# NeptuneHub/AudioMuse-AI

Hardware: AMD Instinct MI355X
Metric: clap_clips_per_sec (higher is better)
Workload: dtype bf16; 1 GPU; model=htsat_clap_student_49M, global_batch=256, seq_len=480000, parallelism=dp1

## Files before the change

audiomuse_amd/config.py:

```python

from __future__ import annotations

import os
from typing import Callable, Dict, Optional

_DB_OVERRIDE_PROVIDER: Optional[Callable[[], Dict[str, str]]] = None


def _env(name: str, default: str) -> str:
    return os.environ.get(name, default)


def _env_int(name: str, default: int) -> int:
    try:
        return int(os.environ.get(name, default))
    except (TypeError, ValueError):
        return default


def _env_float(name: str, default: float) -> float:
    try:
        return float(os.environ.get(name, default))
    except (TypeError, ValueError):
        return default
# ... 253 lines not shown
    "CLUSTERING_STALL_TIMEOUT_MINUTES", 30.0)
TOP_N_ELITES = _env_int("TOP_N_ELITES", 5)
EXPLOITATION_START_FRACTION = _env_float("EXPLOITATION_START_FRACTION", 0.2)
EXPLOITATION_PROBABILITY_CONFIG = _env_float(
    "EXPLOITATION_PROBABILITY_CONFIG", 0.6)
MUTATION_INT_ABS_DELTA = _env_int("MUTATION_INT_ABS_DELTA", 3)
MUTATION_FLOAT_ABS_DELTA = _env_float("MUTATION_FLOAT_ABS_DELTA", 0.25)
MUTATION_KMEANS_COORD_FRACTION = _env_float(
    "MUTATION_KMEANS_COORD_FRACTION", 0.05)
SAMPLING_PERCENTAGE_CHANGE_PER_RUN = _env_float(
    "SAMPLING_PERCENTAGE_CHANGE_PER_RUN", 0.2)
MIN_SONGS_PER_GENRE_FOR_STRATIFICATION = _env_int(
    "MIN_SONGS_PER_GENRE_FOR_STRATIFICATION", 100)
STRATIFIED_SAMPLING_TARGET_PERCENTILE = _env_float(
    "STRATIFIED_SAMPLING_TARGET_PERCENTILE", 50.0)
TOP_K_MOODS_FOR_PURITY_CALCULATION = _env_int(
    "TOP_K_MOODS_FOR_PURITY_CALCULATION", 3)
CLUSTER_NAMING_AI_HISTORY = _env_bool("CLUSTER_NAMING_AI_HISTORY", True)
PLAYLIST_NAME_HISTORY_ROUNDS = _env_int("PLAYLIST_NAME_HISTORY_ROUNDS", 3)

NUM_CLUSTERS_MIN = _env_int("NUM_CLUSTERS_MIN", 2)
NUM_CLUSTERS_MAX = _env_int("NUM_CLUSTERS_MAX", 40)
DBSCAN_EPS_MIN = _env_float("DBSCAN_EPS_MIN", 0.2)
DBSCAN_EPS_MAX = _env_float("DBSCAN_EPS_MAX", 2.5)
DBSCAN_MIN_SAMPLES_MIN = _env_int("DBSCAN_MIN_SAMPLES_MIN", 3)
DBSCAN_MIN_SAMPLES_MAX = _env_int("DBSCAN_MIN_SAMPLES_MAX", 15)
GMM_N_COMPONENTS_MIN = _env_int("GMM_N_COMPONENTS_MIN", 2)
GMM_N_COMPONENTS_MAX = _env_int("GMM_N_COMPONENTS_MAX", 30)
GMM_COVARIANCE_TYPE = _env("GMM_COVARIANCE_TYPE", "diag")
SPECTRAL_N_CLUSTERS_MIN = _env_int("SPECTRAL_N_CLUSTERS_MIN", 2)
SPECTRAL_N_CLUSTERS_MAX = _env_int("SPECTRAL_N_CLUSTERS_MAX", 30)
SPECTRAL_N_NEIGHBORS = _env_int("SPECTRAL_N_NEIGHBORS", 10)
PCA_COMPONENTS_MIN = _env_int("PCA_COMPONENTS_MIN", 0)
PCA_COMPONENTS_MAX = _env_int("PCA_COMPONENTS_MAX", 32)

SCORE_WEIGHT_DIVERSITY = _env_float("SCORE_WEIGHT_DIVERSITY", 2.0)
SCORE_WEIGHT_PURITY = _env_float("SCORE_WEIGHT_PURITY", 1.0)
SCORE_WEIGHT_OTHER_FEATURE_DIVERSITY = _env_float(
    "SCORE_WEIGHT_OTHER_FEATURE_DIVERSITY", 0.0)
SCORE_WEIGHT_OTHER_FEATURE_PURITY = _env_float(
    "SCORE_WEIGHT_OTHER_FEATURE_PURITY", 0.0)
SCORE_WEIGHT_SILHOUETTE = _env_float("SCORE_WEIGHT_SILHOUETTE", 0.0)
SCORE_WEIGHT_DAVIES_BOULDIN = _env_float("SCORE_WEIGHT_DAVIES_BOULDIN", 0.0)
SCORE_WEIGHT_CALINSKI_HARABASZ = _env_float(
    "SCORE_WEIGHT_CALINSKI_HARABASZ", 0.0)

SEM_GROVE_LYRICS_WEIGHT = _env_float("SEM_GROVE_LYRICS_WEIGHT", 0.75)
SEM_GROVE_AUDIO_WEIGHT = _env_float("SEM_GROVE_AUDIO_WEIGHT", 0.25)

ARTIST_GMM_MIN_COMPONENTS = 2
ARTIST_GMM_MAX_COMPONENTS = 10
INDEX_BUILD_WORKERS = _env_int("INDEX_BUILD_WORKERS", 4)

SONIC_FINGERPRINT_HALF_LIFE_DAYS = _env_float("SONIC_FINGERPRINT_HALF_LIFE_DAYS", 30.0)
SONIC_FINGERPRINT_TOP_PLAYED = _env_int("SONIC_FINGERPRINT_TOP_PLAYED", 100)
SONIC_FINGERPRINT_TOP_N_SONGS = _env_int("SONIC_FINGERPRINT_TOP_N_SONGS", 50)
SONIC_FINGERPRINT_NEIGHBORS = _env_int("SONIC_FINGERPRINT_NEIGHBORS", 3)
SONIC_FINGERPRINT_MAX_SONGS_PER_ALBUM = _env_int(
    "SONIC_FINGERPRINT_MAX_SONGS_PER_ALBUM", 0)
SONIC_FINGERPRINT_CRON_PLAYLIST_NAME = _env(
    "SONIC_FINGERPRINT_CRON_PLAYLIST_NAME", "Sonic Fingerprint_automatic")

HYPERBOLIC_SCALE_PERCENTILE = _env_float("HYPERBOLIC_SCALE_PERCENTILE", 95.0)
HYPERBOLIC_DEFAULT_LIMIT = _env_int("HYPERBOLIC_DEFAULT_LIMIT", 50)
HYPERBOLIC_MAX_LIMIT = _env_int("HYPERBOLIC_MAX_LIMIT", 500)
HYPERBOLIC_RADIAL_SPREAD = _env_float("HYPERBOLIC_RADIAL_SPREAD", 0.8)
HYPERBOLIC_CANDIDATE_OVERFETCH = _env_int("HYPERBOLIC_CANDIDATE_OVERFETCH", 4)
HYPERBOLIC_RADIUS_SCALE = _env_float("HYPERBOLIC_RADIUS_SCALE", 1.0)
HYPERBOLIC_RADIUS_PERCENTILE = _env_float("HYPERBOLIC_RADIUS_PERCENTILE", 95.0)
HYPERBOLIC_TARGET_LEAF_SIZE = _env_int("HYPERBOLIC_TARGET_LEAF_SIZE", 200)
HYPERBOLIC_MIN_CLUSTER_SIZE = _env_int("HYPERBOLIC_MIN_CLUSTER_SIZE", 10)
HYPERBOLIC_TREE_WARMUP_DURATION = _env_float(
    "HYPERBOLIC_TREE_WARMUP_DURATION", 300.0)

RADIUS_WALK_BUCKETS = _env_int("RADIUS_WALK_BUCKETS", 10)
RADIUS_INSTRUMENTATION = _env_bool("RADIUS_INSTRUMENTATION", False)

GPU_DTYPE = _env("GPU_DTYPE", "bf16")
CLAP_GPU_BATCH = _env_int("CLAP_GPU_BATCH", 256)
CLAP_FP8_SERVING = _env_bool("AUDIOMUSE_FP8_SERVING", False)
FP8_HIDDEN_ENABLE = _env_bool("AUDIOMUSE_FP8_HIDDEN", False)
FP8_ATTN_ENABLE = _env_bool("AUDIOMUSE_FP8_ATTN", False)
MLP_FUSED_ENABLE = _env_bool("AUDIOMUSE_MLP_FUSED", True)
MERGE_LN_GATHER = _env_bool("AUDIOMUSE_MERGE_LN_GATHER", True)
HIP_REQUIRE_NATIVE = _env_bool("HIP_REQUIRE_NATIVE", True)
RCCL_BUCKET_CAP_MB = _env_int("RCCL_BUCKET_CAP_MB", 64)

AI_PROVIDER = _env("AI_MODEL_PROVIDER", _env("AI_PROVIDER", "none"))
AI_MODEL_NAME = _env("AI_MODEL_NAME", "")
AI_BASE_URL = _env("AI_BASE_URL", "")
AI_API_KEY = _env("AI_API_KEY", "")
AI_MAX_TOOL_CALLS = _env_int("AI_MAX_TOOL_CALLS", 4)
AI_REQUEST_TIMEOUT_SECONDS = _env_float("AI_REQUEST_TIMEOUT_SECONDS", 60.0)
MAX_SONGS_IN_AI_PROMPT = _env_int("MAX_SONGS_IN_AI_PROMPT", 100)
AI_TOOLCALL_TEMPERATURE = _env_float("AI_TOOLCALL_TEMPERATURE", 0.2)
AI_TOOLCALL_TOP_P = _env_float("AI_TOOLCALL_TOP_P", 0.9)
AI_TOOLCALL_TOP_K = _env_int("AI_TOOLCALL_TOP_K", 40)
AI_TOOLCALL_MIN_P = _env_float("AI_TOOLCALL_MIN_P", 0.0)
AI_TOOLCALL_NUM_PREDICT = _env_int("AI_TOOLCALL_NUM_PREDICT", 1024)
OPENAI_API_KEY = _env("OPENAI_API_KEY", "no-key-needed")
OPENAI_MODEL_NAME = _env("OPENAI_MODEL_NAME", "gpt-4o-mini")
OPENAI_SERVER_URL = _env("OPENAI_SERVER_URL", "https://api.openai.com/v1")
OLLAMA_SERVER_URL = _env("OLLAMA_SERVER_URL", "http://127.0.0.1:11434/v1")
OLLAMA_MODEL_NAME = _env("OLLAMA_MODEL_NAME", "llama3.1")
GEMINI_API_KEY = _env("GEMINI_API_KEY", "")
GEMINI_MODEL_NAME = _env("GEMINI_MODEL_NAME", "gemini-2.0-flash")
MISTRAL_API_KEY = _env("MISTRAL_API_KEY", "")
MISTRAL_MODEL_NAME = _env("MISTRAL_MODEL_NAME", "mistral-small-latest")

PLUGINS_ENABLED = _env_bool("PLUGINS_ENABLED", True)
PLUGIN_MAX_DOWNLOAD_MB = _env_int("PLUGIN_MAX_DOWNLOAD_MB", 50)
PLUGIN_ALLOW_PIP = _env_bool("PLUGIN_ALLOW_PIP", False)

JWT_SECRET = _env("AUDIOMUSE_JWT_SECRET", _env("JWT_SECRET", ""))
API_TOKEN = _env("AUDIOMUSE_API_TOKEN", _env("API_TOKEN", ""))
AUTH_ENABLED = _env_bool("AUTH_ENABLED", True)
AUDIOMUSE_USER = _env("AUDIOMUSE_USER", "")
AUDIOMUSE_PASSWORD = _env("AUDIOMUSE_PASSWORD", "")
BEHIND_PROXY = _env_bool("ENABLE_PROXY_FIX",
                         _env_bool("AUDIOMUSE_BEHIND_PROXY", False))
DASHBOARD_BROWSE_PAGE_SIZE = _env_int("DASHBOARD_BROWSE_PAGE_SIZE", 100)
DASHBOARD_BROWSE_MAX_OFFSET = _env_int("DASHBOARD_BROWSE_MAX_OFFSET", 10000)
DASHBOARD_REFRESH_SECONDS = _env_float("DASHBOARD_REFRESH_SECONDS", 60.0)


def set_db_override_provider(provider: Optional[Callable[[], Dict[str, str]]]) -> None:
    global _DB_OVERRIDE_PROVIDER
    _DB_OVERRIDE_PROVIDER = provider


def apply_db_overrides(overrides: Dict[str, str]) -> int:
    import sys

    module = sys.modules[__name__]
    applied = 0
    for key, raw in (overrides or {}).items():
        if not key.isupper() or not hasattr(module, key):
            continue
        current = getattr(module, key)
        try:
            if isinstance(current, bool):
                value = str(raw).strip().lower() in ("1", "true", "yes", "on")
            elif isinstance(current, int):
                value = int(raw)
            elif isinstance(current, float):
                value = float(raw)
            elif isinstance(current, str):
                value = str(raw)
            else:
                continue
        except (TypeError, ValueError):
            continue
        setattr(module, key, value)
        applied += 1
    return applied


def refresh_config() -> None:
    if _DB_OVERRIDE_PROVIDER is not None:
        apply_db_overrides(_DB_OVERRIDE_PROVIDER() or {})


_DEFAULTS_SNAPSHOT: Dict[str, object] = {
    _k: _v for _k, _v in list(globals().items())
    if _k.isupper() and isinstance(_v, (bool, int, float, str))
}
# ... 5 lines not shown
```

audiomuse_amd/models/htsat.py:

```python

from __future__ import annotations

from dataclasses import dataclass
from typing import List, Tuple

import torch
import torch.nn as nn
import torch.nn.functional as F

from audiomuse_amd.ops.attention import window_attention
from audiomuse_amd.ops.norms import FusedLayerNorm


@dataclass
class HTSATConfig:
    n_mels: int = 128
    n_frames: int = 1024
    patch_size: int = 4
    embed_dim: int = 128
    depths: Tuple[int, ...] = (2, 2, 6, 2)
    num_heads: Tuple[int, ...] = (4, 8, 16, 32)
    window: int = 8
    mlp_ratio: float = 4.0
    out_dim: int = 512
# ... 5 lines not shown
    x = x.view(B, H // w, w, W // w, w, C)
    return x.permute(0, 1, 3, 2, 4, 5).reshape(-1, w * w, C)


def window_reverse(win: torch.Tensor, w: int, H: int, W: int) -> torch.Tensor:
    B = win.shape[0] // (H // w * W // w)
    x = win.view(B, H // w, W // w, w, w, -1)
    return x.permute(0, 1, 3, 2, 4, 5).reshape(B, H, W, -1)


class WindowAttention(nn.Module):

    def __init__(self, dim: int, heads: int, window: int):
        super().__init__()
        self.dim = dim
        self.heads = heads
        self.window = window
        self.scale = (dim // heads) ** -0.5
        self.qkv = nn.Linear(dim, dim * 3, bias=True)
        self.proj = nn.Linear(dim, dim)

        n = (2 * window - 1) ** 2
        self.rel_bias = nn.Parameter(torch.zeros(n, heads))
        coords = torch.stack(torch.meshgrid(
            torch.arange(window), torch.arange(window), indexing="ij"))
        flat = coords.flatten(1)
        rel = flat[:, :, None] - flat[:, None, :]
        rel = rel.permute(1, 2, 0) + (window - 1)
        idx = rel[..., 0] * (2 * window - 1) + rel[..., 1]
        self.register_buffer("rel_index", idx, persistent=False)
        nn.init.trunc_normal_(self.rel_bias, std=0.02)

    def full_bias(self) -> torch.Tensor:
        T = self.window * self.window
        bias = self.rel_bias[self.rel_index.view(-1)].view(T, T, self.heads)
        return bias.permute(2, 0, 1).float().contiguous()

    def full_bias_bf16(self) -> torch.Tensor:
        ver = self.rel_bias._version
        cached = getattr(self, "_bias_cache", None)
        if cached is not None and cached[0] == ver \
                and cached[1].device == self.rel_bias.device:
            return cached[1]
        table = self.full_bias().to(torch.bfloat16).contiguous()
        self._bias_cache = (ver, table)
        return table

    def forward(self, x: torch.Tensor, mask: torch.Tensor | None) -> torch.Tensor:
        nW, T, C = x.shape
        qkv = self.qkv(x).reshape(nW, T, 3, self.heads, C // self.heads)
        q, k, v = qkv.permute(2, 0, 3, 1, 4).unbind(0)
        bias = self.full_bias().to(x.dtype)
        out = window_attention(q, k, v, bias, mask, self.scale)
        out = out.transpose(1, 2).reshape(nW, T, C)
        return self.proj(out)


class SwinBlock(nn.Module):
    def __init__(self, dim: int, heads: int, window: int, shift: int, mlp_ratio: float):
        super().__init__()
        self.window = window
        self.shift = shift
        self.norm1 = FusedLayerNorm(dim)
        self.attn = WindowAttention(dim, heads, window)
        self.norm2 = FusedLayerNorm(dim)
        hidden = int(dim * mlp_ratio)
        self.mlp = nn.Sequential(nn.Linear(dim, hidden),
                                 nn.GELU(approximate="tanh"),
                                 nn.Linear(hidden, dim))

    def _fused_available(self, x: torch.Tensor) -> bool:
        if not (x.is_cuda and x.dtype == torch.bfloat16
                and self.mlp[0].weight.dtype == torch.bfloat16
                and not torch.is_grad_enabled()):
            return False
        from audiomuse_amd.ops import _ext
        ext = _ext.native_or_none()
        return ext is not None and hasattr(ext, "window_attn_fwd")

    def _fused_attn_available(self, x: torch.Tensor) -> bool:
        return (self._fused_available(x) and self.window in (4, 8)
                and self.attn.heads % 2 == 0
                and self.attn.dim // self.attn.heads == 32)

    _MLP_FUSED_DIMS = (128,)
    _MLP_FUSED_BM = 128

    def _mlp_half(self, ext, x: torch.Tensor,
                  attn_out: torch.Tensor) -> torch.Tensor:
        from audiomuse_amd import config
        C = x.shape[-1]
        ln_w = self.norm2.weight.to(torch.bfloat16).contiguous()
        ln_b = self.norm2.bias.to(torch.bfloat16).contiguous()
        if (config.MLP_FUSED_ENABLE and C in self._MLP_FUSED_DIMS
                and self.mlp[0].out_features == 4 * C
                and (x.numel() // C) % self._MLP_FUSED_BM == 0):
            return ext.mlp_fused(
                x.contiguous(), attn_out.contiguous(), ln_w, ln_b,
                self.norm2.eps,
                self.mlp[0].weight.contiguous(), self.mlp[0].bias.contiguous(),
                self.mlp[2].weight.contiguous(), self.mlp[2].bias.contiguous())
        x2, xn2 = ext.add_layernorm_bf16(
            x.contiguous(), attn_out.contiguous(), ln_w, ln_b, self.norm2.eps)
        hidden = ext.linear_gelu(xn2, self.mlp[0].weight.contiguous(),
                                 self.mlp[0].bias.contiguous())
        return ext.linear_bias_add(hidden,
                                   self.mlp[2].weight.contiguous(),
                                   self.mlp[2].bias.contiguous(), x2)

    def _eager_attn(self, x: torch.Tensor, H: int, W: int,
                    mask: torch.Tensor | None) -> torch.Tensor:
        B, L, C = x.shape
        x = self.norm1(x).view(B, H, W, C)
        if self.shift:
            x = torch.roll(x, shifts=(-self.shift, -self.shift), dims=(1, 2))
        win = window_partition(x, self.window)
        win = self.attn(win, mask if self.shift else None)
        x = window_reverse(win, self.window, H, W)
        if self.shift:
            x = torch.roll(x, shifts=(self.shift, self.shift), dims=(1, 2))
        return x.view(B, L, C)

    def forward(self, x: torch.Tensor, H: int, W: int,
                mask: torch.Tensor | None) -> torch.Tensor:
        B, L, C = x.shape
        if self._fused_attn_available(x):
            from audiomuse_amd.ops import _ext, fp8
            ext = _ext.require()
            use_fp8 = fp8.serving_enabled() and fp8.available(x.device)
            out = None
            if use_fp8:
                xq, xs = fp8.ln_fp8(self.norm1, x)
                wq, ws = fp8.quantize_weight(self.attn.qkv.weight)
                qkv_bias = self.attn.qkv.bias.to(torch.bfloat16).contiguous()
                if self.window == 8 and fp8.FP8_ATTN[0]:
                    try:
                        qsc, qinv, qamax = fp8.hidden_state(self.attn.qkv,
                                                            x.device)
                        qkv8 = ext.linear_fp8(xq, wq, xs, ws, qkv_bias,
                                              d_inv_scale=qinv)
                        samp = qkv8.reshape(-1)[: 1 << 22]
                        qamax.copy_(samp.float().abs().amax() * qsc)
                        out = ext.window_attn_fp8_fwd(
                            qkv8.view(B, H, W, 3 * C),
                            self.attn.full_bias_bf16(), qsc,
                            self.attn.heads, self.shift, self.attn.scale)
                    except RuntimeError as exc:
                        fp8.FP8_ATTN[0] = False
                        fp8.FP8_ATTN_ERR = str(exc)
                if out is None:
                    qkv = ext.linear_fp8(xq, wq, xs, ws, qkv_bias)
            else:
                xn = self.norm1(x)
                qkv = ext.linear_bias(xn.contiguous(),
                                      self.attn.qkv.weight.contiguous(),
                                      self.attn.qkv.bias.contiguous())
            if out is None:
                attn_fwd = (ext.window_attn_fwd if self.window == 8
                            else ext.window_attn4_fwd)
                out = attn_fwd(
                    qkv.view(B, H, W, 3 * C), self.attn.full_bias_bf16(),
                    self.attn.heads, self.shift, self.attn.scale)
            out = out.view(B, L, C)
            proj = ext.linear_bias(out.contiguous(),
                                   self.attn.proj.weight.contiguous(),
                                   self.attn.proj.bias.contiguous())
            if use_fp8:
                x2, xn2q, xs2 = fp8.add_ln_fp8(self.norm2, x, proj)
                w0q, w0s = fp8.quantize_weight(self.mlp[0].weight)
                b0 = self.mlp[0].bias.to(torch.bfloat16).contiguous()
                if fp8.FP8_HIDDEN[0]:
                    try:
                        hs, hinv, hamax = fp8.hidden_state(self.mlp[0],
                                                           x.device)
                        hidden8 = ext.linear_fp8(xn2q, w0q, xs2, w0s, b0,
                                                 gelu=True,
                                                 d_inv_scale=hinv)
                        samp = hidden8.reshape(-1)[: 1 << 22]
                        hamax.copy_(samp.float().abs().amax() * hs)
                        w2q, w2s = fp8.quantize_weight(self.mlp[2].weight)
                        return ext.linear_fp8(
                            hidden8, w2q, hs, w2s,
                            self.mlp[2].bias.to(torch.bfloat16).contiguous(),
                            resid=x2)
                    except RuntimeError as exc:
                        fp8.FP8_HIDDEN[0] = False
                        fp8.FP8_HIDDEN_ERR = str(exc)
                hidden = ext.linear_fp8(xn2q, w0q, xs2, w0s, b0, gelu=True)
                return ext.linear_bias_add(hidden,
                                           self.mlp[2].weight.contiguous(),
                                           self.mlp[2].bias.contiguous(), x2)
            return self._mlp_half(ext, x, proj)
        if self._fused_available(x):
            from audiomuse_amd.ops import _ext
            ext = _ext.require()
            attn_out = self._eager_attn(x, H, W, mask)
            return self._mlp_half(ext, x, attn_out)
        x = x + self._eager_attn(x, H, W, mask)
        return x + self.mlp(self.norm2(x))


class PatchMerging(nn.Module):

    def __init__(self, dim: int):
        super().__init__()
        self.norm = FusedLayerNorm(4 * dim)
        self.reduction = nn.Linear(4 * dim, 2 * dim, bias=False)

    def _gather_available(self, x: torch.Tensor) -> bool:
        from audiomuse_amd import config
        if not (config.MERGE_LN_GATHER and x.is_cuda
                and x.dtype == torch.bfloat16
                and not torch.is_grad_enabled()
                and 128 < self.norm.normalized_shape[0] <= 4096):
            return False
        from audiomuse_amd.ops import _ext
        ext = _ext.native_or_none()
        return ext is not None and hasattr(ext, "merge_layernorm_bf16")

    def forward(self, x: torch.Tensor, H: int, W: int) -> torch.Tensor:
        B, L, C = x.shape
        if self._gather_available(x):
            from audiomuse_amd.ops import _ext
            y = _ext.require().merge_layernorm_bf16(
                x.contiguous().view(B, H, W, C),
                self.norm.weight.to(torch.bfloat16).contiguous(),
                self.norm.bias.to(torch.bfloat16).contiguous(),
                self.norm.eps)
            return self.reduction(y)
        x = x.view(B, H // 2, 2, W // 2, 2, C)
        x = x.permute(0, 1, 3, 4, 2, 5).reshape(B, (H // 2) * (W // 2),
                                                4 * C)
        return self.reduction(self.norm(x))

# ... 82 lines not shown
```

audiomuse_amd/ops/csrc/bindings.cpp:

```cpp
#include <hip/hip_runtime.h>
#include <torch/extension.h>

#include <algorithm>
#include <vector>

#include <c10/hip/HIPStream.h>

namespace audiomuse {
void launch_mel_fwd(const float* audio, float* out, const float* window,
                    const float2* twiddle, const int* mel_rowptr,
                    const int* mel_bin, const float* mel_w, int B, int T,
                    int n_frames, int hop, int n_mels, int n_fft, int center,
                    int log_mode, int quant16, hipStream_t stream);
void launch_ivf_scan(int dtype_code, int metric, const void* query,
                     const float* qnorm, const void* data,
                     const float* row_norm, const int* probe,
                     const int* cell_off, const long long* cand_off,
                     float* out_dist, int* out_row, int Q, int d, int nprobe,
                     long long cap, hipStream_t stream);
void launch_ivf_scan_sel(int dtype_code, int metric, const void* query,
                         const float* qnorm, const void* data,
                         const float* row_norm, const int* probe,
                         const int* sel_rows, const int* sel_off,
                         const long long* cand_off, float* out_dist,
                         int* out_row, int Q, int d, int nprobe, long long cap,
                         hipStream_t stream);
void launch_ivf_scan_topk(int dtype_code, int metric, const void* query,
                          const float* qnorm, const void* data,
                          const float* row_norm, const int* probe,
                          const int* off, const int* sel_rows,
                          const int* skip_row, float* out_dist, int* out_row,
                          int Q, int S, int K, int d, int nprobe,
                          hipStream_t stream);
void launch_umap_epoch(const float* E, float* out, const int* idx,
                       const int* thr, const int* in_off, const int* in_edge,
                       const int* in_thr, int n, int k, int n_in, int neg,
                       float alpha, float a, float b, unsigned int seed,
                       unsigned int epoch, hipStream_t stream);
void launch_path_relax(const float* dist_in, const int* pred_in,
                       float* dist_out, int* pred_out, const int* idx,
                       const float* w, const int* in_off, const int* in_edge,
                       const unsigned char* allowed, int* changed, int B,
                       int n, int k, int n_in, int legs_inner,
                       hipStream_t stream);
void launch_path_walk(const float* dist, const int* pred, const int* src,
                      const int* dst, int* out, int* count, int B, int n,
                      int T1, int legs_inner, hipStream_t stream);
void launch_layernorm_bf16(const void* x, void* y, const void* w,
                           const void* b, long long n_rows, int dim, float eps,
                           hipStream_t stream);
void launch_add_layernorm_bf16(const void* x, const void* in2, void* sum_out,
                               void* y, const void* w, const void* b,
                               long long n_rows, int dim, float eps,
                               hipStream_t stream);
void launch_layernorm_bf16_fp8_impl(const void* x, void* y8, const void* w,
                                    const void* b, const void* in2,
                                    void* sum_out, const float* q_scale,
                                    float* q_amax, long long n_rows, int dim,
                                    float eps, hipStream_t stream);
void launch_mfma_probe(const void* A, const void* B, float* D,
                       hipStream_t stream);
void launch_window_attn4(const void* qkv, void* out, const void* bias,
                         int Bn, int H, int W, int C, int heads, int shift,
                         float scale, hipStream_t stream);
void launch_window_attn(const void* qkv, void* out, const void* bias, int Bn,
                        int H, int W, int C, int heads, int shift, float scale,
                        hipStream_t stream);
void launch_merge_layernorm_bf16(const void* x, void* y, const void* w,
                                 const void* b, int Bn, int H, int W, int C,
                                 float eps, hipStream_t stream);
void launch_mlp_fused_c128(const void* x, const void* proj, const void* ln_w,
                           const void* ln_b, const void* W1, const void* b1,
                           const void* W2, const void* b2, void* out,
                           long long M, float eps, hipStream_t stream);
void launch_window_attn_fp8(const void* qkv, void* out, const void* bias,
                            const void* qs_ptr, int Bn, int H, int W, int C,
                            int heads, int shift, float sm_scale,
                            hipStream_t stream);
void launch_fp_align(const int* words, const long long* off, const int* pairs,
                     int* out, long long W, int F, long long P, int max_offset,
                     int min_words, int lds_words, hipStream_t stream);
}

#define AM_CHECK(x, msg) TORCH_CHECK(x, msg)
#define AM_CHECK_GPU_F32_CONTIG(t)                                   \
  TORCH_CHECK(t.is_cuda() && t.scalar_type() == at::kFloat &&        \
                  t.is_contiguous(),                                 \
              #t " must be a contiguous float32 GPU tensor")

static torch::Tensor mel_fwd(torch::Tensor audio, torch::Tensor window,
                             torch::Tensor twiddle, torch::Tensor mel_rowptr,
                             torch::Tensor mel_bin, torch::Tensor mel_w,
                             int64_t hop, int64_t n_fft, bool center,
                             int64_t log_mode, bool quant16) {
  AM_CHECK_GPU_F32_CONTIG(audio);
  AM_CHECK_GPU_F32_CONTIG(window);
  AM_CHECK_GPU_F32_CONTIG(mel_w);
  AM_CHECK(audio.dim() == 2, "audio must be (B, T)");
  AM_CHECK(twiddle.is_cuda() && twiddle.is_contiguous() &&
               twiddle.scalar_type() == at::kFloat &&
               twiddle.numel() == n_fft,
           "twiddle must be (n_fft/2, 2) float32 on GPU");
  AM_CHECK(mel_rowptr.is_cuda() && mel_rowptr.scalar_type() == at::kInt &&
               mel_bin.scalar_type() == at::kInt,
           "CSR index tensors must be int32 on GPU");
  AM_CHECK(n_fft == 256 || n_fft == 512 || n_fft == 1024 || n_fft == 2048 ||
               n_fft == 4096,
           "n_fft must be a power of two in [256, 4096]");

  const int64_t B = audio.size(0);
  const int64_t T = audio.size(1);
  const int64_t n_mels = mel_rowptr.numel() - 1;
  const int64_t n_frames =
      center ? (1 + T / hop) : (1 + (T - n_fft) / hop);
  AM_CHECK(n_frames >= 1, "audio too short for one frame");

  auto out = torch::empty({B, n_mels, n_frames}, audio.options());
  auto stream = c10::hip::getCurrentHIPStream();
  audiomuse::launch_mel_fwd(
      audio.data_ptr<float>(), out.data_ptr<float>(), window.data_ptr<float>(),
      reinterpret_cast<const float2*>(twiddle.data_ptr<float>()),
      mel_rowptr.data_ptr<int>(), mel_bin.data_ptr<int>(),
      mel_w.data_ptr<float>(), (int)B, (int)T, (int)n_frames, (int)hop,
      (int)n_mels, (int)n_fft, center ? 1 : 0, (int)log_mode, quant16 ? 1 : 0,
      stream.stream());
  C10_HIP_CHECK(hipGetLastError());
  return out;
}

static void ivf_scan(int64_t dtype_code, int64_t metric, torch::Tensor query,
                     torch::Tensor qnorm, torch::Tensor data,
                     torch::Tensor row_norm, torch::Tensor probe,
                     torch::Tensor cell_off, torch::Tensor cand_off,
                     torch::Tensor out_dist, torch::Tensor out_row,
                     int64_t dim_pad) {
  AM_CHECK(query.is_cuda() && data.is_cuda(), "ivf_scan needs GPU tensors");
  AM_CHECK(probe.scalar_type() == at::kInt && cell_off.scalar_type() == at::kInt,
           "probe/cell_off must be int32");
  AM_CHECK(cand_off.scalar_type() == at::kLong, "cand_off must be int64");
  AM_CHECK(out_dist.is_contiguous() && out_row.is_contiguous(),
           "outputs must be contiguous");
  const int Q = probe.size(0);
  const int nprobe = probe.size(1);
  const long long cap = out_dist.size(1);
  auto stream = c10::hip::getCurrentHIPStream();
  audiomuse::launch_ivf_scan(
      (int)dtype_code, (int)metric, query.data_ptr(), qnorm.data_ptr<float>(),
      data.data_ptr(), row_norm.data_ptr<float>(), probe.data_ptr<int>(),
      cell_off.data_ptr<int>(),
      reinterpret_cast<const long long*>(cand_off.data_ptr<int64_t>()),
      out_dist.data_ptr<float>(), out_row.data_ptr<int>(), Q, (int)dim_pad,
      nprobe, cap, stream.stream());
  C10_HIP_CHECK(hipGetLastError());
}

static void ivf_scan_sel(int64_t dtype_code, int64_t metric,
                         torch::Tensor query, torch::Tensor qnorm,
// ... 441 lines not shown
  return y8;
}

static std::vector<torch::Tensor> add_layernorm_bf16_fp8(
    torch::Tensor x, torch::Tensor other, torch::Tensor w, torch::Tensor b,
    double eps, torch::Tensor scale, torch::Tensor amax) {
  AM_CHECK(x.is_cuda() && x.scalar_type() == at::kBFloat16 && x.is_contiguous(),
           "x must be contiguous bf16 on GPU");
  AM_CHECK(other.is_contiguous() && other.sizes() == x.sizes() &&
               other.scalar_type() == at::kBFloat16,
           "other must match x");
  const int dim = x.size(-1);
  AM_CHECK(dim % 4 == 0 && dim <= 4096, "dim must be /4 and <= 4096");
  auto sum = torch::empty_like(x);
  auto y8 = torch::empty(x.sizes(), x.options().dtype(at::kFloat8_e4m3fn));
  const long long n_rows = x.numel() / dim;
  auto stream = c10::hip::getCurrentHIPStream();
  audiomuse::launch_layernorm_bf16_fp8_impl(
      x.data_ptr(), y8.data_ptr(), w.data_ptr(), b.data_ptr(),
      other.data_ptr(), sum.data_ptr(), scale.data_ptr<float>(),
      amax.data_ptr<float>(), n_rows, dim, (float)eps, stream.stream());
  C10_HIP_CHECK(hipGetLastError());
  return {sum, y8};
}

static torch::Tensor merge_layernorm_bf16(torch::Tensor x, torch::Tensor w,
                                          torch::Tensor b, double eps) {
  AM_CHECK(x.is_cuda() && x.scalar_type() == at::kBFloat16 &&
               x.is_contiguous() && x.dim() == 4,
           "x must be (B, H, W, C) bf16 contiguous GPU");
  const int64_t Bn = x.size(0), H = x.size(1), W = x.size(2), C = x.size(3);
  AM_CHECK(H % 2 == 0 && W % 2 == 0, "H, W must be even");
  AM_CHECK(C % 4 == 0 && 4 * C > 128 && 4 * C <= 4096,
           "C must be a multiple of 4 with 128 < 4C <= 4096");
  AM_CHECK(w.is_cuda() && b.is_cuda() && w.is_contiguous() &&
               b.is_contiguous() && w.scalar_type() == at::kBFloat16 &&
               b.scalar_type() == at::kBFloat16 && w.numel() == 4 * C &&
               b.numel() == 4 * C,
           "w/b must be contiguous bf16 of size 4C");
  auto y = torch::empty({Bn, (H / 2) * (W / 2), 4 * C}, x.options());
  auto stream = c10::hip::getCurrentHIPStream();
  audiomuse::launch_merge_layernorm_bf16(x.data_ptr(), y.data_ptr(),
                                         w.data_ptr(), b.data_ptr(), (int)Bn,
                                         (int)H, (int)W, (int)C, (float)eps,
                                         stream.stream());
  C10_HIP_CHECK(hipGetLastError());
  return y;
}

static torch::Tensor mlp_fused(torch::Tensor x, torch::Tensor proj,
                               torch::Tensor ln_w, torch::Tensor ln_b,
                               double eps, torch::Tensor w1, torch::Tensor b1,
                               torch::Tensor w2, torch::Tensor b2) {
  auto ok = [](const torch::Tensor& t) {
    return t.is_cuda() && t.scalar_type() == at::kBFloat16 &&
           t.is_contiguous();
  };
  AM_CHECK(ok(x) && ok(proj) && ok(ln_w) && ok(ln_b) && ok(w1) && ok(b1) &&
               ok(w2) && ok(b2),
           "all inputs must be contiguous bf16 GPU tensors");
  const int64_t C = x.size(-1);
  AM_CHECK(C == 128, "mlp_fused is built for C = 128");
  const int64_t M = x.numel() / C;
  AM_CHECK(M > 0 && M % 128 == 0, "token count must be a multiple of 128");
  AM_CHECK(M / 128 < (1ll << 31), "too many tokens for one launch");
  AM_CHECK(proj.sizes() == x.sizes(), "proj must match x");
  AM_CHECK(ln_w.numel() == C && ln_b.numel() == C, "LN weight/bias size");
  AM_CHECK(w1.dim() == 2 && w1.size(0) == 4 * C && w1.size(1) == C &&
               b1.numel() == 4 * C,
           "w1 must be (4C, C), b1 (4C)");
  AM_CHECK(w2.dim() == 2 && w2.size(0) == C && w2.size(1) == 4 * C &&
               b2.numel() == C,
           "w2 must be (C, 4C), b2 (C)");
  auto out = torch::empty_like(x);
  auto stream = c10::hip::getCurrentHIPStream();
  audiomuse::launch_mlp_fused_c128(
      x.data_ptr(), proj.data_ptr(), ln_w.data_ptr(), ln_b.data_ptr(),
      w1.data_ptr(), b1.data_ptr(), w2.data_ptr(), b2.data_ptr(),
      out.data_ptr(), (long long)M, (float)eps, stream.stream());
  C10_HIP_CHECK(hipGetLastError());
  return out;
}

static torch::Tensor fp_align(torch::Tensor words, torch::Tensor off,
                              torch::Tensor pairs, int64_t max_offset,
                              int64_t min_words, int64_t lds_words) {
  AM_CHECK(words.is_cuda() && off.is_cuda() && pairs.is_cuda(),
           "fp_align needs GPU tensors");
  AM_CHECK(words.get_device() == off.get_device() &&
               words.get_device() == pairs.get_device(),
           "words, off and pairs must be on one device");
  AM_CHECK(words.scalar_type() == at::kInt && words.dim() == 1 &&
               words.is_contiguous(),
           "words must be a contiguous (W,) int32 tensor");
  AM_CHECK(off.scalar_type() == at::kLong && off.dim() == 1 &&
               off.is_contiguous() && off.numel() >= 1,
           "off must be a contiguous (F+1,) int64 tensor");
  AM_CHECK(pairs.scalar_type() == at::kInt && pairs.dim() == 2 &&
               pairs.size(1) == 2 && pairs.is_contiguous(),
           "pairs must be a contiguous (P, 2) int32 tensor");
  AM_CHECK(max_offset >= 0 && max_offset <= 1024,
           "max_offset must be in [0, 1024]");
  AM_CHECK(min_words >= 1, "min_words must be >= 1");
  AM_CHECK(lds_words >= 1 && lds_words <= 4096,
           "lds_words must be in [1, 4096]");
  const int64_t F = off.numel() - 1;
  const int64_t P = pairs.size(0);
  AM_CHECK(F < (1ll << 31) && P < (1ll << 31),
           "fp_align is limited to F, P < 2^31");
  auto out = torch::empty({P, 3}, pairs.options());
  if (P == 0) return out;
  auto stream = c10::hip::getCurrentHIPStream();
  audiomuse::launch_fp_align(
      words.data_ptr<int>(),
      reinterpret_cast<const long long*>(off.data_ptr<int64_t>()),
      pairs.data_ptr<int>(), out.data_ptr<int>(), (long long)words.numel(),
      (int)F, (long long)P, (int)max_offset,
      (int)std::min<int64_t>(min_words, 1 << 30), (int)lds_words,
      stream.stream());
  C10_HIP_CHECK(hipGetLastError());
  return out;
}

void register_gemm_gelu(pybind11::module_& m);

PYBIND11_MODULE(TORCH_EXTENSION_NAME, m) {
  m.doc() = "AudioMuse-AMD native CDNA4 kernels";
  register_gemm_gelu(m);
  m.def("add_layernorm_bf16", &add_layernorm_bf16,
        "Fused residual add + LayerNorm: returns (x+other, LN(x+other))");
  m.def("layernorm_bf16_fp8", &layernorm_bf16_fp8,
        "LayerNorm with fused e4m3 quantize (delayed scale + amax)");
  m.def("add_layernorm_bf16_fp8", &add_layernorm_bf16_fp8,
        "Residual add + LN with fused e4m3 quantize: (sum bf16, y fp8)");
  m.def("mfma_probe", &mfma_probe, "16x16x32 bf16 MFMA layout probe");
  m.def("window_attn_fp8_fwd", &window_attn_fp8_fwd,
        "fused shifted-window attention, fp8-ingest QKV (e4m3 + device "
        "dequant scale), bf16 MFMAs/out");
  m.def("window_attn_fwd", &window_attn_fwd,
        "Fused shifted-window attention (qkv BHW3C bf16, bias, heads, "
        "shift, scale) -> (B,H,W,C)");
  m.def("merge_layernorm_bf16", &merge_layernorm_bf16,
        "LayerNorm over 2x2-merged patches gathered from (B,H,W,C): "
        "(x, w, b, eps) -> (B, H/2*W/2, 4C)");
  m.def("mlp_fused", &mlp_fused,
        "x2 = x + proj; out = x2 + W2 gelu_tanh(W1 LN(x2) + b1) + b2 in one "
        "launch, C = 128 (x, proj, ln_w, ln_b, eps, w1, b1, w2, b2)");
  m.def("window_attn4_fwd", &window_attn4_fwd,
        "Fused 4x4-window attention for stage 4 (qkv BHW3C bf16, "
        "bias (heads,16,16), heads, shift, scale) -> (B,H,W,C)");
  m.def("layernorm_bf16", &layernorm_bf16,
        "Fused LayerNorm forward, bf16 in/out, fp32 stats (x, w, b, eps)");
  m.def("mel_fwd", &mel_fwd,
        "Fused STFT+mel+log spectrogram (audio, window, twiddle, rowptr, "
        "bin, w, hop, n_fft, center, log_mode)");
  m.def("ivf_scan", &ivf_scan,
        "IVF probed-cell distance scan (dtype, metric, query, qnorm, data, "
        "row_norm, probe, cell_off, cand_off, out_dist, out_row, dim_pad)");
  m.def("ivf_scan_sel", &ivf_scan_sel,
        "IVF probed-cell scan over a row selection (dtype, metric, query, "
        "qnorm, data, row_norm, probe, sel_rows, sel_off, cand_off, out_dist, "
        "out_row, dim_pad)");
  m.def("ivf_scan_topk", &ivf_scan_topk,
        "IVF probed-cell scan that keeps the K best per (query, split) "
        "(dtype, metric, query, qnorm, data, row_norm, probe, cell_off, "
        "sel_rows|None, sel_off|None, skip_row|None, out_dist (Q,S,K), "
        "out_row (Q,S,K), dim_pad)");
  m.def("umap_epoch", &umap_epoch,
        "One epoch of the 2-D map layout, one launch (E, out, idx, thr, "
        "in_off, in_edge, in_thr, alpha, a, b, seed, epoch, neg)");
  m.def("path_relax", &path_relax,
        "One Bellman-Ford sweep over the symmetrised kNN graph for up to 8 "
        "legs (pull pass, ping-pong buffers)");
  m.def("path_walk", &path_walk,
        "Follow shortest-path predecessors from each target to its source");
  m.def("fp_align", &fp_align,
        "Best alignment of fingerprint pairs (words int32 (W,), off int64 "
        "(F+1,), pairs int32 (P, 2), max_offset, min_words, lds_words) -> "
        "(P, 3) int32 (bits, n, offset)");
  m.attr("gfx_arch") = "gfx950";
}
```

setup.py:

```python

import os

from setuptools import setup

os.environ.setdefault("PYTORCH_ROCM_ARCH", "gfx950")

from torch.utils.cpp_extension import BuildExtension, CUDAExtension

CSRC = os.path.join("audiomuse_amd", "ops", "csrc")

sources = [
    os.path.join(CSRC, "bindings.cpp"),
    os.path.join(CSRC, "gemm_gelu.cpp"),
    os.path.join(CSRC, "mel.hip"),
]
for extra in ("distance.hip", "kmeans.hip", "attention.hip", "norms.hip",
              "mlp_fused.hip", "layout.hip", "fingerprint.hip", "path.hip"):
    p = os.path.join(CSRC, extra)
    if os.path.exists(p):
        sources.append(p)

setup(
    name="audiomuse-amd",
    version="0.1.0",
    packages=["audiomuse_amd"],
    ext_modules=[
        CUDAExtension(
            "audiomuse_amd._C",
            sources,
            libraries=["hipblaslt"],
            extra_compile_args={
                "cxx": ["-O3", "-std=c++17"],
                "nvcc": ["-O3", "-std=c++17"],
            },
        )
    ],
    cmdclass={"build_ext": BuildExtension},
)
```

Baseline: 10750 clips/s.

## Fuse LN, QKV, window attention and projection into one kernel for stage 1

```diff
diff --git a/audiomuse_amd/config.py b/audiomuse_amd/config.py
--- a/audiomuse_amd/config.py
+++ b/audiomuse_amd/config.py
@@ -359,6 +359,7 @@
 FP8_HIDDEN_ENABLE = _env_bool("AUDIOMUSE_FP8_HIDDEN", False)
 FP8_ATTN_ENABLE = _env_bool("AUDIOMUSE_FP8_ATTN", False)
 MLP_FUSED_ENABLE = _env_bool("AUDIOMUSE_MLP_FUSED", True)
+ATTN_FUSED_ENABLE = _env_bool("AUDIOMUSE_ATTN_FUSED", True)
 MERGE_LN_GATHER = _env_bool("AUDIOMUSE_MERGE_LN_GATHER", True)
 HIP_REQUIRE_NATIVE = _env_bool("HIP_REQUIRE_NATIVE", True)
 RCCL_BUCKET_CAP_MB = _env_int("RCCL_BUCKET_CAP_MB", 64)
diff --git a/audiomuse_amd/models/htsat.py b/audiomuse_amd/models/htsat.py
--- a/audiomuse_amd/models/htsat.py
+++ b/audiomuse_amd/models/htsat.py
@@ -111,6 +111,14 @@
         return (self._fused_available(x) and self.window in (4, 8)
                 and self.attn.heads % 2 == 0
                 and self.attn.dim // self.attn.heads == 32)
+
+    def _attn_block_fused_applies(self, ext, H: int, W: int) -> bool:
+        from audiomuse_amd import config
+        return (config.ATTN_FUSED_ENABLE and self.window == 8
+                and self.attn.dim == 128 and self.attn.heads == 4
+                and self.shift in (0, 4)
+                and H % 8 == 0 and W % 8 == 0
+                and hasattr(ext, "attn_block_fused"))
 
     _MLP_FUSED_DIMS = (128,)
     _MLP_FUSED_BM = 128
@@ -179,6 +187,18 @@
                         fp8.FP8_ATTN_ERR = str(exc)
                 if out is None:
                     qkv = ext.linear_fp8(xq, wq, xs, ws, qkv_bias)
+            elif self._attn_block_fused_applies(ext, H, W):
+                proj = ext.attn_block_fused(
+                    x.contiguous().view(B, H, W, C),
+                    self.norm1.weight.to(torch.bfloat16).contiguous(),
+                    self.norm1.bias.to(torch.bfloat16).contiguous(),
+                    self.norm1.eps,
+                    self.attn.qkv.weight.contiguous(),
+                    self.attn.qkv.bias.contiguous(),
+                    self.attn.proj.weight.contiguous(),
+                    self.attn.proj.bias.contiguous(),
+                    self.attn.full_bias_bf16(), self.shift, self.attn.scale)
+                return self._mlp_half(ext, x, proj.view(B, L, C))
             else:
                 xn = self.norm1(x)
                 qkv = ext.linear_bias(xn.contiguous(),
diff --git a/audiomuse_amd/ops/csrc/attn_fused.hip b/audiomuse_amd/ops/csrc/attn_fused.hip
--- /dev/null
+++ b/audiomuse_amd/ops/csrc/attn_fused.hip
@@ -0,0 +1,306 @@
+
+#include <hip/hip_runtime.h>
+
+namespace audiomuse {
+
+namespace {
+
+typedef __bf16 bf16x8 __attribute__((ext_vector_type(8)));
+typedef __bf16 bf16x4 __attribute__((ext_vector_type(4)));
+typedef float f32x4 __attribute__((ext_vector_type(4)));
+
+constexpr int AF_C = 128;
+constexpr int AF_T = 64;
+constexpr int AF_TILE = AF_T * AF_C;
+
+__device__ __forceinline__ int af_off(int row, int ch) {
+  return row * AF_C + ((ch ^ (row & 15)) << 3);
+}
+
+__device__ __forceinline__ int af_off_c4(int row, int c) {
+  return af_off(row, c >> 3) + (c & 7);
+}
+
+__device__ __forceinline__ bf16x8 af_pack(const f32x4 lo, const f32x4 hi) {
+  bf16x8 r;
+#pragma unroll
+  for (int j = 0; j < 4; ++j) {
+    r[j] = (__bf16)lo[j];
+    r[4 + j] = (__bf16)hi[j];
+  }
+  return r;
+}
+
+__device__ __forceinline__ f32x4 af_mfma(const bf16x8 a, const bf16x8 b,
+                                         const f32x4 c) {
+  return __builtin_amdgcn_mfma_f32_16x16x32_bf16(a, b, c, 0, 0, 0);
+}
+
+}
+
+__global__ __launch_bounds__(256, 2) void attn_fused_c128_kernel(
+    const __bf16* __restrict__ x,
+    const __bf16* __restrict__ ln_w,
+    const __bf16* __restrict__ ln_b,
+    const __bf16* __restrict__ qkv_w,
+    const __bf16* __restrict__ qkv_b,
+    const __bf16* __restrict__ proj_w,
+    const __bf16* __restrict__ proj_b,
+    const __bf16* __restrict__ bias,
+    __bf16* __restrict__ out,
+    int H, int W, int shift, float scale, float eps) {
+  __shared__ __attribute__((aligned(16))) __bf16 lds[2 * AF_TILE];
+  __bf16* bufA = lds;
+  __bf16* bufB = lds + AF_TILE;
+
+  const int tid = threadIdx.x;
+  const int lane = tid & 63;
+  const int wave = tid >> 6;
+  const int l16 = lane & 15;
+  const int g = lane >> 4;
+
+  const int nWw = W >> 3;
+  const int nWh = H >> 3;
+  const int win = blockIdx.x;
+  const int b = win / (nWh * nWw);
+  const int wrem = win - b * (nWh * nWw);
+  const int wh = wrem / nWw;
+  const int ww = wrem - wh * nWw;
+
+  auto src_of = [&](int t, int& si, int& sj, int& wrap) {
+    const int ri = t >> 3, ci = t & 7;
+    int gi = wh * 8 + ri + shift;
+    int gj = ww * 8 + ci + shift;
+    const int wr = gi >= H;
+    const int wc = gj >= W;
+    si = wr ? gi - H : gi;
+    sj = wc ? gj - W : gj;
+    wrap = (wr << 1) | wc;
+  };
+
+  unsigned long long wrap_r_mask, wrap_c_mask;
+  {
+    int si, sj, wrap;
+    src_of(lane, si, sj, wrap);
+    wrap_r_mask = __ballot(wrap & 2);
+    wrap_c_mask = __ballot(wrap & 1);
+  }
+
+  const int ch = tid & 15;
+  long long row_off[4];
+  {
+    bf16x8 xv[4];
+#pragma unroll
+    for (int i = 0; i < 4; ++i) {
+      int si, sj, wrap;
+      src_of(16 * i + (tid >> 4), si, sj, wrap);
+      row_off[i] = (((long long)b * H + si) * W + sj) * AF_C + ch * 8;
+      xv[i] = *(const bf16x8*)(x + row_off[i]);
+    }
+    const bf16x8 lw = *(const bf16x8*)(ln_w + ch * 8);
+    const bf16x8 lb = *(const bf16x8*)(ln_b + ch * 8);
+#pragma unroll
+    for (int i = 0; i < 4; ++i) {
+      float sum = 0.0f;
+#pragma unroll
+      for (int j = 0; j < 8; ++j) sum += (float)xv[i][j];
+#pragma unroll
+      for (int d = 1; d < 16; d <<= 1) sum += __shfl_xor(sum, d, 64);
+      const float mean = sum / AF_C;
+      float var = 0.0f;
+#pragma unroll
+      for (int j = 0; j < 8; ++j) {
+        const float dv = (float)xv[i][j] - mean;
+        var += dv * dv;
+      }
+#pragma unroll
+      for (int d = 1; d < 16; d <<= 1) var += __shfl_xor(var, d, 64);
+      const float rstd = rsqrtf(var / AF_C + eps);
+      bf16x8 y;
+#pragma unroll
+      for (int j = 0; j < 8; ++j)
+        y[j] = (__bf16)((((float)xv[i][j] - mean) * rstd) * (float)lw[j] +
+                        (float)lb[j]);
+      *(bf16x8*)(bufA + af_off(16 * i + (tid >> 4), ch)) = y;
+    }
+  }
+  __syncthreads();
+
+  const int h = wave;
+  bf16x8 xn[4][4];
+#pragma unroll
+  for (int tr = 0; tr < 4; ++tr)
+#pragma unroll
+    for (int ks = 0; ks < 4; ++ks)
+      xn[tr][ks] = *(const bf16x8*)(bufA + af_off(16 * tr + l16, 4 * ks + g));
+
+  bf16x8 qk[2][4];
+#pragma unroll
+  for (int which = 0; which < 2; ++which) {
+    f32x4 acc[2][4];
+#pragma unroll
+    for (int dt = 0; dt < 2; ++dt) {
+      const int feat = which * AF_C + h * 32 + dt * 16;
+      const __bf16* wrow = qkv_w + (feat + l16) * AF_C + 8 * g;
+      bf16x8 wf[4];
+#pragma unroll
+      for (int ks = 0; ks < 4; ++ks) wf[ks] = *(const bf16x8*)(wrow + 32 * ks);
+      const bf16x4 bb = *(const bf16x4*)(qkv_b + feat + 4 * g);
+#pragma unroll
+      for (int tr = 0; tr < 4; ++tr) {
+        f32x4 a = {(float)bb[0], (float)bb[1], (float)bb[2], (float)bb[3]};
+#pragma unroll
+        for (int ks = 0; ks < 4; ++ks) a = af_mfma(wf[ks], xn[tr][ks], a);
+        acc[dt][tr] = a;
+      }
+    }
+#pragma unroll
+    for (int tr = 0; tr < 4; ++tr)
+      qk[which][tr] = af_pack(acc[0][tr], acc[1][tr]);
+  }
+
+  bf16x8 vf[2][2];
+#pragma unroll
+  for (int dt = 0; dt < 2; ++dt) {
+    const int feat = 2 * AF_C + h * 32 + dt * 16;
+    const __bf16* wrow = qkv_w + (feat + l16) * AF_C + 8 * g;
+    bf16x8 wf[4];
+#pragma unroll
+    for (int ks = 0; ks < 4; ++ks) wf[ks] = *(const bf16x8*)(wrow + 32 * ks);
+    const float bv = (float)qkv_b[feat + l16];
+    f32x4 acc[4];
+#pragma unroll
+    for (int tr = 0; tr < 4; ++tr) {
+      f32x4 a = {bv, bv, bv, bv};
+#pragma unroll
+      for (int ks = 0; ks < 4; ++ks) a = af_mfma(xn[tr][ks], wf[ks], a);
+      acc[tr] = a;
+    }
+    vf[dt][0] = af_pack(acc[0], acc[1]);
+    vf[dt][1] = af_pack(acc[2], acc[3]);
+  }
+
+  bf16x8 wp[2][4];
+#pragma unroll
+  for (int ct = 0; ct < 2; ++ct)
+#pragma unroll
+    for (int ks = 0; ks < 4; ++ks)
+      wp[ct][ks] = *(const bf16x8*)(proj_w +
+                                    (32 * wave + 16 * ct + l16) * AF_C +
+                                    32 * ks + 8 * g);
+
+  f32x4 st[4][4];
+#pragma unroll
+  for (int tc = 0; tc < 4; ++tc)
+#pragma unroll
+    for (int tr = 0; tr < 4; ++tr) {
+      const f32x4 z = {0.f, 0.f, 0.f, 0.f};
+      st[tc][tr] = af_mfma(qk[1][tc], qk[0][tr], z);
+    }
+
+  bf16x8 pf[4][2];
+#pragma unroll
+  for (int tr = 0; tr < 4; ++tr) {
+    const int tq = 16 * tr + l16;
+    const int qwrap = (int)((((wrap_r_mask >> tq) & 1ull) << 1) |
+                            ((wrap_c_mask >> tq) & 1ull));
+    const __bf16* brow = bias + (h * 64 + tq) * 64 + 4 * g;
+    float m = -1e30f;
+#pragma unroll
+    for (int tc = 0; tc < 4; ++tc) {
+      const bf16x4 bb = *(const bf16x4*)(brow + 16 * tc);
+#pragma unroll
+      for (int reg = 0; reg < 4; ++reg) {
+        const int tk = 16 * tc + 4 * g + reg;
+        const int kwrap = (int)((((wrap_r_mask >> tk) & 1ull) << 1) |
+                                ((wrap_c_mask >> tk) & 1ull));
+        float v = st[tc][tr][reg] * scale + (float)bb[reg];
+        if (shift && qwrap != kwrap) v = -1e30f;
+        st[tc][tr][reg] = v;
+        m = fmaxf(m, v);
+      }
+    }
+    m = fmaxf(m, __shfl_xor(m, 16, 64));
+    m = fmaxf(m, __shfl_xor(m, 32, 64));
+    float sum = 0.0f;
+#pragma unroll
+    for (int tc = 0; tc < 4; ++tc)
+#pragma unroll
+      for (int reg = 0; reg < 4; ++reg) {
+        const float e = __expf(st[tc][tr][reg] - m);
+        st[tc][tr][reg] = e;
+        sum += e;
+      }
+    sum += __shfl_xor(sum, 16, 64);
+    sum += __shfl_xor(sum, 32, 64);
+    const float inv = __frcp_rn(sum + 1e-20f);
+#pragma unroll
+    for (int tc = 0; tc < 4; ++tc)
+#pragma unroll
+      for (int reg = 0; reg < 4; ++reg) st[tc][tr][reg] *= inv;
+    pf[tr][0] = af_pack(st[0][tr], st[1][tr]);
+    pf[tr][1] = af_pack(st[2][tr], st[3][tr]);
+  }
+
+#pragma unroll
+  for (int dt = 0; dt < 2; ++dt)
+#pragma unroll
+    for (int tr = 0; tr < 4; ++tr) {
+      f32x4 o = {0.f, 0.f, 0.f, 0.f};
+      o = af_mfma(vf[dt][0], pf[tr][0], o);
+      o = af_mfma(vf[dt][1], pf[tr][1], o);
+      bf16x4 ob;
+#pragma unroll
+      for (int reg = 0; reg < 4; ++reg) ob[reg] = (__bf16)o[reg];
+      *(bf16x4*)(bufB + af_off_c4(16 * tr + l16, 32 * h + 16 * dt + 4 * g)) =
+          ob;
+    }
+  __syncthreads();
+
+  bf16x4 pb[2];
+#pragma unroll
+  for (int ct = 0; ct < 2; ++ct)
+    pb[ct] = *(const bf16x4*)(proj_b + 32 * wave + 16 * ct + 4 * g);
+#pragma unroll
+  for (int tr = 0; tr < 4; ++tr) {
+    bf16x8 of[4];
+#pragma unroll
+    for (int ks = 0; ks < 4; ++ks)
+      of[ks] = *(const bf16x8*)(bufB + af_off(16 * tr + l16, 4 * ks + g));
+#pragma unroll
+    for (int ct = 0; ct < 2; ++ct) {
+      f32x4 a = {(float)pb[ct][0], (float)pb[ct][1], (float)pb[ct][2],
+                 (float)pb[ct][3]};
+#pragma unroll
+      for (int ks = 0; ks < 4; ++ks) a = af_mfma(wp[ct][ks], of[ks], a);
+      bf16x4 ob;
+#pragma unroll
+      for (int reg = 0; reg < 4; ++reg) ob[reg] = (__bf16)a[reg];
+      *(bf16x4*)(bufA +
+                 af_off_c4(16 * tr + l16, 32 * wave + 16 * ct + 4 * g)) = ob;
+    }
+  }
+  __syncthreads();
+
+#pragma unroll
+  for (int i = 0; i < 4; ++i)
+    *(bf16x8*)(out + row_off[i]) =
+        *(const bf16x8*)(bufA + af_off(16 * i + (tid >> 4), ch));
+}
+
+void launch_attn_fused_c128(const void* x, const void* ln_w, const void* ln_b,
+                            const void* qkv_w, const void* qkv_b,
+                            const void* proj_w, const void* proj_b,
+                            const void* bias, void* out, int Bn, int H, int W,
+                            int shift, float scale, float eps,
+                            hipStream_t stream) {
+  const unsigned n_windows = (unsigned)Bn * (H >> 3) * (W >> 3);
+  hipLaunchKernelGGL(attn_fused_c128_kernel, dim3(n_windows), dim3(256), 0,
+                     stream, (const __bf16*)x, (const __bf16*)ln_w,
+                     (const __bf16*)ln_b, (const __bf16*)qkv_w,
+                     (const __bf16*)qkv_b, (const __bf16*)proj_w,
+                     (const __bf16*)proj_b, (const __bf16*)bias,
+                     (__bf16*)out, H, W, shift, scale, eps);
+}
+
+}
diff --git a/audiomuse_amd/ops/csrc/bindings.cpp b/audiomuse_amd/ops/csrc/bindings.cpp
--- a/audiomuse_amd/ops/csrc/bindings.cpp
+++ b/audiomuse_amd/ops/csrc/bindings.cpp
@@ -73,6 +73,12 @@
                            const void* ln_b, const void* W1, const void* b1,
                            const void* W2, const void* b2, void* out,
                            long long M, float eps, hipStream_t stream);
+void launch_attn_fused_c128(const void* x, const void* ln_w, const void* ln_b,
+                            const void* qkv_w, const void* qkv_b,
+                            const void* proj_w, const void* proj_b,
+                            const void* bias, void* out, int Bn, int H, int W,
+                            int shift, float scale, float eps,
+                            hipStream_t stream);
 void launch_window_attn_fp8(const void* qkv, void* out, const void* bias,
                             const void* qs_ptr, int Bn, int H, int W, int C,
                             int heads, int shift, float sm_scale,
@@ -680,6 +686,57 @@
   return out;
 }
 
+static torch::Tensor attn_block_fused(
+    torch::Tensor x, torch::Tensor ln_w, torch::Tensor ln_b, double eps,
+    torch::Tensor qkv_w, torch::Tensor qkv_b, torch::Tensor proj_w,
+    torch::Tensor proj_b, torch::Tensor bias, int64_t shift, double scale,
+    c10::optional<torch::Tensor> out) {
+  auto ok = [](const torch::Tensor& t) {
+    return t.is_cuda() && t.scalar_type() == at::kBFloat16 &&
+           t.is_contiguous();
+  };
+  AM_CHECK(ok(x) && ok(ln_w) && ok(ln_b) && ok(qkv_w) && ok(qkv_b) &&
+               ok(proj_w) && ok(proj_b) && ok(bias),
+           "all inputs must be contiguous bf16 GPU tensors");
+  AM_CHECK(x.dim() == 4, "x must be (B, H, W, C)");
+  const int64_t Bn = x.size(0), H = x.size(1), W = x.size(2), C = x.size(3);
+  AM_CHECK(C == 128, "attn_block_fused is built for C = 128");
+  AM_CHECK(H > 0 && W > 0 && H % 8 == 0 && W % 8 == 0,
+           "H, W must be multiples of 8");
+  AM_CHECK(shift == 0 || shift == 4, "shift must be 0 or 4");
+  AM_CHECK(Bn > 0 && Bn * (H / 8) * (W / 8) < (1ll << 31) &&
+               H < (1 << 30) && W < (1 << 30),
+           "too many windows for one launch");
+  AM_CHECK(ln_w.numel() == C && ln_b.numel() == C, "LN weight/bias size");
+  AM_CHECK(qkv_w.dim() == 2 && qkv_w.size(0) == 3 * C && qkv_w.size(1) == C &&
+               qkv_b.numel() == 3 * C,
+           "qkv_w must be (3C, C), qkv_b (3C)");
+  AM_CHECK(proj_w.dim() == 2 && proj_w.size(0) == C && proj_w.size(1) == C &&
+               proj_b.numel() == C,
+           "proj_w must be (C, C), proj_b (C)");
+  AM_CHECK(bias.dim() == 3 && bias.size(0) == 4 && bias.size(1) == 64 &&
+               bias.size(2) == 64,
+           "bias must be (4, 64, 64): 4 heads of 32");
+  torch::Tensor o;
+  if (out.has_value()) {
+    o = *out;
+    AM_CHECK(ok(o) && o.sizes() == x.sizes() &&
+                 o.get_device() == x.get_device(),
+             "out must be a contiguous bf16 GPU tensor shaped like x");
+    AM_CHECK(o.data_ptr() != x.data_ptr(), "out must not alias x");
+  } else {
+    o = torch::empty_like(x);
+  }
+  auto stream = c10::hip::getCurrentHIPStream();
+  audiomuse::launch_attn_fused_c128(
+      x.data_ptr(), ln_w.data_ptr(), ln_b.data_ptr(), qkv_w.data_ptr(),
+      qkv_b.data_ptr(), proj_w.data_ptr(), proj_b.data_ptr(), bias.data_ptr(),
+      o.data_ptr(), (int)Bn, (int)H, (int)W, (int)shift, (float)scale,
+      (float)eps, stream.stream());
+  C10_HIP_CHECK(hipGetLastError());
+  return o;
+}
+
 static torch::Tensor fp_align(torch::Tensor words, torch::Tensor off,
                               torch::Tensor pairs, int64_t max_offset,
                               int64_t min_words, int64_t lds_words) {
@@ -744,6 +801,15 @@
   m.def("mlp_fused", &mlp_fused,
         "x2 = x + proj; out = x2 + W2 gelu_tanh(W1 LN(x2) + b1) + b2 in one "
         "launch, C = 128 (x, proj, ln_w, ln_b, eps, w1, b1, w2, b2)");
+  m.def("attn_block_fused", &attn_block_fused,
+        "LN -> QKV -> 8x8 window attention -> proj in one launch, C = 128, "
+        "4 heads; returns proj (x, ln_w, ln_b, eps, qkv_w, qkv_b, proj_w, "
+        "proj_b, bias (4,64,64), shift, scale, out=None) -> (B,H,W,128)",
+        pybind11::arg("x"), pybind11::arg("ln_w"), pybind11::arg("ln_b"),
+        pybind11::arg("eps"), pybind11::arg("qkv_w"), pybind11::arg("qkv_b"),
+        pybind11::arg("proj_w"), pybind11::arg("proj_b"),
+        pybind11::arg("bias"), pybind11::arg("shift"), pybind11::arg("scale"),
+        pybind11::arg("out") = pybind11::none());
   m.def("window_attn4_fwd", &window_attn4_fwd,
         "Fused 4x4-window attention for stage 4 (qkv BHW3C bf16, "
         "bias (heads,16,16), heads, shift, scale) -> (B,H,W,C)");
diff --git a/setup.py b/setup.py
--- a/setup.py
+++ b/setup.py
@@ -15,7 +15,8 @@
     os.path.join(CSRC, "mel.hip"),
 ]
 for extra in ("distance.hip", "kmeans.hip", "attention.hip", "norms.hip",
-              "mlp_fused.hip", "layout.hip", "fingerprint.hip", "path.hip"):
+              "mlp_fused.hip", "attn_fused.hip", "layout.hip",
+              "fingerprint.hip", "path.hip"):
     p = os.path.join(CSRC, extra)
     if os.path.exists(p):
         sources.append(p)
```

Measured after the change: 11880 clips/s (median of 6 runs). 10.5% higher.
